# lazear/sage

Hardware: NVIDIA H100
Metric: spectra/sec (higher is better)
Workload: dtype f32

## Files before the change

sage_b200/csrc/device_common.cuh:

```cuda
#pragma once
#include <cuda_runtime.h>
#include <stdint.h>

namespace sb {

constexpr int K_MAX = 128;
constexpr uint32_t NARROW_CAP = 8192;
constexpr int PRELIM_THREADS = 256;
constexpr int SCORE_THREADS = 128;
#ifndef SAGE_B200_SCORE_MIN_CTAS
#define SAGE_B200_SCORE_MIN_CTAS 10
#endif
constexpr int SCORE_MIN_CTAS = SAGE_B200_SCORE_MIN_CTAS;
#ifndef SAGE_B200_SCORE_TILE
#define SAGE_B200_SCORE_TILE 1024
#endif
#ifndef SAGE_B200_SCORE_UNROLL
#define SAGE_B200_SCORE_UNROLL 1
#endif
#ifndef SAGE_B200_SCORE_MIN_CTAS_SPLIT
#define SAGE_B200_SCORE_MIN_CTAS_SPLIT 11
#endif
constexpr int SCORE_MIN_CTAS_SPLIT = SAGE_B200_SCORE_MIN_CTAS_SPLIT;
constexpr uint32_t SCORE_UNROLL = SAGE_B200_SCORE_UNROLL;
constexpr uint32_t SCORE_TILE = SAGE_B200_SCORE_TILE;
constexpr int MAX_KINDS = 6;
constexpr uint32_t WARPQ_CAP = 1024;
constexpr int WARPQ_WARPS = 2;
constexpr int WARPQ_MIN_CTAS = 24;
constexpr uint32_t PEP_LUT_CELLS = 65536;
constexpr uint32_t BUCKET_LUT_CELLS = 32768;

constexpr float PROTON = 1.0072764f;
constexpr float NEUTRON = 1.00335f;

struct Tol { int kind; float lo, hi; };

__device__ __forceinline__ int f32_key(float x) {
    int b = __float_as_int(x);
    return b ^ (int)(((unsigned)(b >> 31)) >> 1);
}

__device__ __forceinline__ float div_const_rn(float x, float c, float rc) {
    const float ax = fabsf(x);
    if (ax >= 1e-20f && ax <= 1e30f) {
        const float q0 = __fmul_rn(x, rc);
        return __fmaf_rn(__fmaf_rn(-q0, c, x), rc, q0);
    }
    return __fdiv_rn(x, c);
}

__device__ __forceinline__ void tol_bounds(const Tol& t, float c, float& lo, float& hi) {
    if (t.kind == 0) {
        lo = __fadd_rn(c, div_const_rn(__fmul_rn(c, t.lo), 1000000.0f, 1.0f / 1000000.0f));
        hi = __fadd_rn(c, div_const_rn(__fmul_rn(c, t.hi), 1000000.0f, 1.0f / 1000000.0f));
    } else if (t.kind == 1) {
        lo = __fadd_rn(c, div_const_rn(__fmul_rn(c, t.lo), 100.0f, 1.0f / 100.0f));
        hi = __fadd_rn(c, div_const_rn(__fmul_rn(c, t.hi), 100.0f, 1.0f / 100.0f));
    } else {
        lo = __fadd_rn(c, t.lo);
        hi = __fadd_rn(c, t.hi);
    }
// ... 65 lines not shown
    uint8_t mode;
};

struct QueryHits {
    uint32_t n;
    uint32_t default_run;
    uint32_t matched_peaks;
    uint32_t scored_candidates;
};

__device__ __forceinline__ uint32_t smem_u32(const void* p) { return (uint32_t)__cvta_generic_to_shared(p); }
__device__ __forceinline__ void mbar_init(uint64_t* bar, uint32_t count) {
    asm volatile("mbarrier.init.shared::cta.b64 [%0], %1;" ::"r"(smem_u32(bar)), "r"(count) : "memory");
    asm volatile("fence.mbarrier_init.release.cluster;" ::: "memory");
}
__device__ __forceinline__ void mbar_arrive_expect_tx(uint64_t* bar, uint32_t bytes) {
    asm volatile("mbarrier.arrive.expect_tx.shared::cta.b64 _, [%0], %1;" ::"r"(smem_u32(bar)), "r"(bytes) : "memory");
}
__device__ __forceinline__ void bulk_copy_g2s(void* dst_smem, const void* src_gmem, uint32_t bytes, uint64_t* bar) {
    asm volatile("cp.async.bulk.shared::cluster.global.mbarrier::complete_tx::bytes [%0], [%1], %2, [%3];" ::"r"(smem_u32(dst_smem)), "l"(src_gmem), "r"(bytes),
                 "r"(smem_u32(bar))
                 : "memory");
}
__device__ __forceinline__ void mbar_wait(uint64_t* bar, uint32_t parity) {
    uint32_t done = 0;
    while (!done) {
        asm volatile(
            "{\n\t.reg .pred p;\n\tmbarrier.try_wait.parity.shared::cta.b64 p, [%1], %2;\n\tselp.u32 %0, 1, 0, p;\n\t}"
            : "=r"(done)
            : "r"(smem_u32(bar)), "r"(parity)
            : "memory");
    }
}

struct ReplaySlot { unsigned long long off; uint32_t item, n_list, state , k; };

enum { C_TASKS = 0, C_PAGES, C_ENTRIES, C_MATCHED, C_CANDS, C_PEPFLOATS, C_PSMS, C_QUERIES, C_WIDE, C_MAXPOT, C_WORK, C_ERR, C_PEPQ, C_PEPFALLBACK, C_WSLOT, C_WOVERFLOW, C_FRAGS,
       C_NLIST , C_NCTA , C_NLIST_NEED ,
       C_HITS , C_COUNT };

struct DbView {
    const uint2* frag;
    const float* bucket_min;
    const float* pep_mono;
    const uint32_t* ion_off;
    const float* ions;
    const uint8_t* pep_len;
    const uint8_t* pep_flags;
    const uint8_t* pep_missed;
    uint32_t n_pep, n_bucket, bucket_size, n_kinds;
    uint32_t min_ion_index;
    uint32_t pep_centric_ok;
    uint32_t nterm_mask;
    const uint16_t* page_grid;
    uint32_t grid_shift, grid_n;
    const uint32_t* bucket_lut;
    float blut_base, blut_inv_w;
    const uint32_t* pep_lut;
    float plut_base, plut_inv_w;
    uint64_t n_frag;
    uint8_t kinds[MAX_KINDS];
};

struct WideIndexView {
    const uint2* frag;
    const uint64_t* blk_off;
// ... 54 lines not shown
```

sage_b200/csrc/kernels.cuh:

```cuda
#pragma once
#include <type_traits>

#include "device_common.cuh"
#include "glibc_log.cuh"

#ifndef SAGE_B200_RARE_NOINLINE
#define SAGE_B200_RARE_NOINLINE 0
#endif
#if SAGE_B200_RARE_NOINLINE
#define SB_RARE __noinline__
#else
#define SB_RARE __forceinline__
#endif

namespace sb {

__device__ __forceinline__ uint32_t pep_partition(const DbView& db, float x, bool le) {
    uint32_t lo = 0, hi = db.n_pep;
    if (db.pep_lut != nullptr) {
        const float t = (x - db.plut_base) * db.plut_inv_w;
        if (t == t) {
            const int c = (int)fminf(fmaxf(floorf(t), -2.0f), (float)PEP_LUT_CELLS + 2.0f);
            lo = __ldg(db.pep_lut + min(max(c - 1, 0), (int)PEP_LUT_CELLS));
            hi = __ldg(db.pep_lut + min(max(c + 2, 0), (int)PEP_LUT_CELLS));
// ... 229 lines not shown
}

__device__ __forceinline__ void index_probe(const DbView& db, const QueryDesc& q, float flo, float fhi, uint32_t* cnt32, uint32_t& matched, uint32_t& pages,
                                            uint32_t& entries) {
    uint32_t bl, br;
    bucket_range(db, flo, fhi, bl, br);
    for (uint32_t page = bl; page < br; page++) {
        const uint64_t pbase = (uint64_t)page * db.bucket_size;
        const uint64_t pend = min(pbase + db.bucket_size, db.n_frag);
        const uint2* slice = db.frag + pbase;
        const uint32_t pn = (uint32_t)(pend - pbase);
        const uint32_t pp = page_lower_bound_dir(db, page, slice, pn, q.pre_lo);
        const uint32_t il = pp == 0 ? 0 : pp - 1;
        uint32_t e = pp;
        for (; e < pn; e++) {
            const uint2 f = __ldg(&slice[e]);
            if (f.x > q.pre_hi) break;
            const float fmz = __uint_as_float(f.y);
            if (f.x >= q.eff_lo && f.x <= q.eff_hi && fmz >= flo && fmz <= fhi) {
                const uint32_t idx = f.x - q.pre_lo;
                atomicAdd(&cnt32[idx >> 1], 1u << ((idx & 1) * 16));
                matched++;
            }
        }
        pages++;
        entries += e - il;
    }
}

#ifndef SAGE_B200_WALK_SOLO
#define SAGE_B200_WALK_SOLO 8
#endif
constexpr uint32_t WALK_SOLO = SAGE_B200_WALK_SOLO;
__device__ __forceinline__ void block_probe_warp(const WideIndexView& nv, const QueryDesc& q, uint32_t b0, uint32_t b1, bool act, float flo, float fhi,
                                                 uint32_t* cnt32, uint32_t& matched) {
    const uint32_t lane = threadIdx.x & 31;
    const float tt = (flo - nv.base) * nv.inv_w;
    const int c = tt > 1.0f ? (int)fminf(tt, (float)(nv.cells - 1)) - 1 : 0;
    for (uint32_t blk = b0; blk <= b1; blk++) {
        const uint64_t base = __ldg(nv.blk_off + blk);
        const uint32_t cnt = (uint32_t)(__ldg(nv.blk_off + blk + 1) - base);
        const uint2* fr = nv.frag + base;
        uint32_t e = cnt;
        if (act) {
            e = __ldg(nv.lut + (size_t)blk * (nv.cells + 1) + c);
            for (uint32_t k = 0; k < WALK_SOLO && e < cnt; k++, e++) {
                const uint2 f = __ldg(fr + e);
                const float fmz = __uint_as_float(f.y);
                if (fmz > fhi) { e = cnt; break; }
                if (fmz >= flo && f.x >= q.eff_lo && f.x <= q.eff_hi) {
                    const uint32_t idx = f.x - q.pre_lo;
                    atomicAdd(&cnt32[idx >> 1], 1u << ((idx & 1) * 16));
                    matched++;
                }
            }
        }
        uint32_t pend = __ballot_sync(0xffffffffu, e < cnt);
        while (pend) {
            const int src = __ffs(pend) - 1;
            pend &= pend - 1;
            const uint32_t e0 = __shfl_sync(0xffffffffu, e, src);
            const float lo_s = __shfl_sync(0xffffffffu, flo, src), hi_s = __shfl_sync(0xffffffffu, fhi, src);
            for (uint32_t pos = e0; pos < cnt; pos += 32) {
                const uint32_t i = pos + lane;
                bool stop = i >= cnt;
                if (!stop) {
                    const uint2 f = __ldg(fr + i);
                    const float fmz = __uint_as_float(f.y);
                    stop = fmz > hi_s;
                    if (!stop && fmz >= lo_s && f.x >= q.eff_lo && f.x <= q.eff_hi) {
                        const uint32_t idx = f.x - q.pre_lo;
                        atomicAdd(&cnt32[idx >> 1], 1u << ((idx & 1) * 16));
                        matched++;
                    }
                }
                if (__any_sync(0xffffffffu, stop)) break;
            }
        }
    }
}

__device__ __forceinline__ void narrow_cta_query(const DbView& db, const ScorerView& sc, const BatchView& b, uint32_t pmax, uint64_t* nlist, uint32_t item,
                                                 float* bounds_smem, const WideIndexView& nv) {
    __shared__ uint32_t cnt32[NARROW_CAP / 2 + 1];
    __shared__ uint32_t s_warp[40];
    ReplaySlot* const nslots = b.nslots;
    const uint32_t s = item / sc.qmax;
    const QueryDesc q = b.queries[item];
    const uint32_t tid = threadIdx.x, lane = tid & 31, warp = tid >> 5, nwarps = PRELIM_THREADS / 32;
    const uint32_t p0 = b.peak_off[s], np = b.peak_off[s + 1] - p0;
    const uint32_t nwords = (q.potential + 1) >> 1;
    for (uint32_t i = tid; i < nwords; i += PRELIM_THREADS) cnt32[i] = 0;
    __shared__ unsigned long long s_loff;
    if (tid == 0 && q.potential > sc.kparam) s_loff = atomicAdd(b.counters + C_NLIST, (unsigned long long)q.potential);

    const uint32_t nfc = q.nfc;
    const uint32_t ntask = np * nfc;
    uint32_t my_matched = 0, my_pages = 0, my_entries = 0;
    __shared__ LutParams s_lp[8];
    bool pep_path = q.mode == 3 && np > 0 && np < 65536 && nfc <= 8;
    float* const bnd = bounds_smem;
    uint16_t* const luts = reinterpret_cast<uint16_t*>(bounds_smem + 2 * (size_t)nfc * pmax);
    if (pep_path) {
        for (uint32_t t = tid; t < ntask; t += PRELIM_THREADS) {
            const uint32_t c = t / np, p = t - c * np;
            const float mass = __fmul_rn(__ldg(b.masses + p0 + p), (float)(c + 1));
            float flo, fhi;
            tol_bounds(sc.fragment_tol, mass, flo, fhi);
            bnd[(2 * c) * pmax + p] = flo;
            bnd[(2 * c + 1) * pmax + p] = fhi;
        }
// ... 40 lines not shown
                            const float f = __ldg(src + j);
                            for (uint32_t c = 0; c < nfc; c++) {
                                const float* lo_c = bnd + (2 * c) * pmax;
                                const float* hi_c = lo_c + pmax;
                                const LutParams LP = s_lp[c];
                                uint32_t a = lut_start(LP, luts + (2 * c) * LUT_CELLS, f);
                                while (a < np && lo_c[a] <= f) a++;
                                uint32_t bb = lut_start(LP, luts + (2 * c + 1) * LUT_CELLS, f);
                                while (bb < a && hi_c[bb] < f) bb++;
                                c_here += a - min(bb, a);
                            }
                        }
                    }
                }
                for (int o = 16; o > 0; o >>= 1) c_here += __shfl_down_sync(0xffffffffu, c_here, o);
                if (lane == 0 && c_here) {
                    const uint32_t idx = pep - q.pre_lo;
                    atomicAdd(&cnt32[idx >> 1], (c_here & 0xFFFFu) << ((idx & 1) * 16));
                    my_matched += c_here;
                }
            }
        }
    } else if (nv.frag != nullptr) {
        const uint32_t blk0 = q.pre_lo / nv.block, blk1 = min(q.pre_hi, db.n_pep - 1) / nv.block;
        for (uint32_t t0 = warp * 32; t0 < ntask; t0 += PRELIM_THREADS) {
            const uint32_t t = t0 + lane;
            const bool act = t < ntask;
            float flo = 0.0f, fhi = 0.0f;
            if (act) {
                const uint32_t p = t / nfc, fc = t - p * nfc + 1;
                const float mass = __fmul_rn(__ldg(b.masses + p0 + p), (float)fc);
                tol_bounds(sc.fragment_tol, mass, flo, fhi);
            }
            block_probe_warp(nv, q, blk0, blk1, act, flo, fhi, cnt32, my_matched);
        }
    } else {
        for (uint32_t t = tid; t < ntask; t += PRELIM_THREADS) {
            const uint32_t p = t / nfc, fc = t - p * nfc + 1;
            const float mass = __fmul_rn(__ldg(b.masses + p0 + p), (float)fc);
            float flo, fhi;
            tol_bounds(sc.fragment_tol, mass, flo, fhi);
            index_probe(db, q, flo, fhi, cnt32, my_matched, my_pages, my_entries);
        }
    }
    __shared__ uint32_t s_red[3][PRELIM_THREADS / 32];
    {
        uint32_t a = my_matched, p = my_pages, en = my_entries;
        for (int o = 16; o > 0; o >>= 1) {
            a += __shfl_down_sync(0xffffffffu, a, o);
            p += __shfl_down_sync(0xffffffffu, p, o);
            en += __shfl_down_sync(0xffffffffu, en, o);
        }
        if (lane == 0) { s_red[0][warp] = a; s_red[1][warp] = p; s_red[2][warp] = en; }
    }
    __syncthreads();
    uint32_t matched_total = 0;
    for (uint32_t w = 0; w < nwarps; w++) matched_total += s_red[0][w];
    if (tid == 0) {
        uint32_t pages_total = 0, entries_total = 0;
        for (uint32_t w = 0; w < nwarps; w++) { pages_total += s_red[1][w]; entries_total += s_red[2][w]; }
        atomicAdd(b.counters + C_TASKS, (unsigned long long)ntask);
        if (pages_total) atomicAdd(b.counters + C_PAGES, (unsigned long long)pages_total);
        if (entries_total) atomicAdd(b.counters + C_ENTRIES, (unsigned long long)entries_total);
        atomicAdd(b.counters + C_MATCHED, (unsigned long long)matched_total);
    }
    QueryHits* h = b.hits + item;
    if (matched_total == 0) {
// ... 65 lines not shown
    const uint32_t total = (uint32_t)min(b.counters[C_NCTA], (unsigned long long)b.n * sc.qmax);
    for (uint32_t i = blockIdx.x; i < total; i += gridDim.x) {
        narrow_cta_query(db, sc, b, pmax, nlist, b.cta_items[i], bounds_smem, nv);
        __syncthreads();
    }
}

template <bool BLK>
__global__ void __launch_bounds__(WARPQ_WARPS * 32, WARPQ_MIN_CTAS) k_prelim_narrow_warp(DbView db, ScorerView sc, BatchView b, uint64_t* nlist, uint32_t s_lo,
                                                                                                uint32_t s_hi, WideIndexView nv) {
    __shared__ uint32_t cnt_all[WARPQ_WARPS][WARPQ_CAP / 2];
    if (b.counters[C_COUNT + blockIdx.y] == 0ull) return;
    const uint32_t lane = threadIdx.x & 31, warp = threadIdx.x >> 5;
    const uint32_t pos = blockIdx.x * WARPQ_WARPS + warp;
    if (pos >= b.n) return;
    const uint32_t s = b.order ? b.order[pos] : pos;
    if (s < s_lo || s >= s_hi) return;
    const uint32_t item = s * sc.qmax + blockIdx.y;
    const QueryDesc q = b.queries[item];
    if (q.mode != 4) return;
    uint32_t* const cnt32 = cnt_all[warp];
    const uint32_t n = q.potential, k = min(n, sc.kparam);
    for (uint32_t i = lane; i < (n + 1) >> 1; i += 32) cnt32[i] = 0;
    unsigned long long loff = 0;
    if (n > k) {
        if (lane == 0) loff = atomicAdd(b.counters + C_NLIST, (unsigned long long)n);
        loff = __shfl_sync(0xffffffffu, loff, 0);
    }
    __syncwarp();
    const uint32_t p0 = b.peak_off[s], np = b.peak_off[s + 1] - p0;
    const uint32_t nfc = q.nfc, ntask = np * nfc;
    uint32_t matched = 0, pages = 0, entries = 0;
    const uint32_t blk0 = BLK ? q.pre_lo / nv.block : 0u, blk1 = BLK ? min(q.pre_hi, db.n_pep - 1) / nv.block : 0u;
    for (uint32_t t0 = 0; t0 < ntask; t0 += 32) {
        const uint32_t t = t0 + lane;
        const bool act = t < ntask;
        float flo = 0.0f, fhi = 0.0f;
        if (act) {
            const uint32_t p = t / nfc, fc = t - p * nfc + 1;
            const float mass = __fmul_rn(__ldg(b.masses + p0 + p), (float)fc);
            tol_bounds(sc.fragment_tol, mass, flo, fhi);
        }
        if (BLK) block_probe_warp(nv, q, blk0, blk1, act, flo, fhi, cnt32, matched);
        else if (act) index_probe(db, q, flo, fhi, cnt32, matched, pages, entries);
    }
    for (int o = 16; o > 0; o >>= 1) {
        matched += __shfl_xor_sync(0xffffffffu, matched, o);
        pages += __shfl_xor_sync(0xffffffffu, pages, o);
        entries += __shfl_xor_sync(0xffffffffu, entries, o);
    }
    __syncwarp();
    if (lane == 0) {
        atomicAdd(b.counters + C_TASKS, (unsigned long long)ntask);
        if (pages) atomicAdd(b.counters + C_PAGES, (unsigned long long)pages);
        if (entries) atomicAdd(b.counters + C_ENTRIES, (unsigned long long)entries);
        if (matched) atomicAdd(b.counters + C_MATCHED, (unsigned long long)matched);
    }
    QueryHits* h = b.hits + item;
    ReplaySlot* slot = b.nslots + item;
    if (matched == 0 || (n > k && loff + n > b.nlist_cap)) {
        if (lane == 0) { h->n = 0; h->default_run = n; h->matched_peaks = 0; h->scored_candidates = 0; }
        return;
    }
    auto cnt = [&](uint32_t i) -> uint32_t { return (cnt32[i >> 1] >> ((i & 1) * 16)) & 0xFFFFu; };
    uint32_t nzc = 0;
    uint64_t* dst = n <= k ? b.hit_keys + (size_t)item * sc.kparam : nlist + loff;
    for (uint32_t i = lane; i < k; i += 32) {
        const uint32_t c = cnt(i);
        nzc += c != 0;
        dst[i] = c ? prescore_key(c, q.pre_lo + i, q.charge, q.iso) : PRESCORE_DEFAULT;
    }
    uint32_t wbase = k;
    for (uint32_t base = k; base < n; base += 32) {
        const uint32_t i = base + lane;
        const uint32_t c = i < n ? cnt(i) : 0;
        nzc += c != 0;
// ... 915 lines not shown
    float term[SCORE_TILE];
    float inten[SCORE_TILE];
    uint32_t mask[SCORE_TILE / 32];
    uint16_t hits[SCORE_TILE];
    uint16_t lut[SPEC_LUT_CELLS];
    uint32_t scan[SCORE_THREADS / 32];
    unsigned long long hit_base;
    uint32_t hit_room;
};

__device__ __forceinline__ uint32_t kind_index(uint32_t ki, uint32_t nions) {
    uint32_t kind = ki >= nions;
    uint32_t idx = ki - (kind ? nions : 0);
    while (idx >= nions) { idx -= nions; kind++; }
    return kind << 13 | idx;
}

__device__ __forceinline__ bool fast_task(float ion, uint32_t fc, float tlo, float thi, const SpecView& sp, const uint16_t* lut, const float* pm, float& mz,
                                          uint32_t& idx) {
    const float q3 = __fmul_rn(ion, 1.0f / 3.0f);
    const float third = __fmaf_rn(__fmaf_rn(-q3, 3.0f, ion), 1.0f / 3.0f, q3);
    mz = fc == 1 ? ion : (fc == 2 ? __fmul_rn(ion, 0.5f) : third);
    const float pl = __fmul_rn(mz, tlo), ph = __fmul_rn(mz, thi);
    const float ql = __fmul_rn(pl, 1.0f / 1000000.0f), qh = __fmul_rn(ph, 1.0f / 1000000.0f);
    const float lo = __fadd_rn(mz, __fmaf_rn(__fmaf_rn(-ql, 1000000.0f, pl), 1.0f / 1000000.0f, ql));
    const float hi = __fadd_rn(mz, __fmaf_rn(__fmaf_rn(-qh, 1000000.0f, ph), 1.0f / 1000000.0f, qh));
    const float tt = __fmul_rn(__fsub_rn(lo, sp.lp.base), sp.lp.inv_w);
    const int cc = tt > 1.0f ? (int)fminf(tt, (float)(SPEC_LUT_CELLS - 1)) - 1 : 0;
    idx = lut[cc];
    while (pm[idx] < lo) idx++;
    return pm[idx] <= hi;
}

template <bool FAST, bool SPLIT>
__device__ __forceinline__ void score_candidates_flat(const DbView& db, const ScorerView& sc, const uint64_t* cur, uint32_t ncand, const SpecView& sp,
                                                      ScoreTile& S, ScoreRec* recs, const SplitOut& so, uint32_t spec) {
    const uint32_t tid = threadIdx.x, lane = tid & 31, warp = tid >> 5, nwarps = SCORE_THREADS / 32;
    constexpr uint32_t tile = SCORE_TILE;
    uint64_t key = 0;
    uint32_t L = 0, nions = 0, nfc = 1, total = 0, ion_off = 0;
    if (tid < ncand) {
        key = cur[tid];
        const uint32_t pep = key_peptide(key);
        L = __ldg(db.pep_len + pep);
        nions = L - 1;
        nfc = max_fragment_charge(sc.max_fragment_charge_opt, key_charge(key)) - 1;
        total = nions * nfc * db.n_kinds;
        ion_off = __ldg(db.ion_off + pep);
    }
    uint32_t incl = total;
#pragma unroll
    for (int o = 1; o < 32; o <<= 1) {
        const uint32_t v = __shfl_up_sync(0xffffffffu, incl, o);
        if (lane >= (uint32_t)o) incl += v;
    }
    if (lane == 31) S.scan[warp] = incl;
    __syncthreads();
    uint32_t base = incl - total, T = 0;
#pragma unroll
    for (uint32_t w = 0; w < nwarps; w++) {
        const uint32_t x = S.scan[w];
        if (w < warp) base += x;
        T += x;
    }
    if (tid < ncand) { CandHdr h; h.ion_off = ion_off; h.base = base; h.next = base + total; h.nions = (uint16_t)nions; h.nfc = (uint8_t)nfc; h.pad = 0; S.hdr[tid] = h; }
    if (tid == 0) { CandHdr h; h.ion_off = 0; h.base = T; h.next = 0xFFFFFFFFu; h.nions = 0; h.nfc = 1; h.pad = 0; S.hdr[ncand] = h; }
    uint32_t hcnt = 0, hits_before = 0;
    if (SPLIT && tid == 0) {
        const unsigned long long hb = atomicAdd(so.counters + C_HITS, (unsigned long long)T);
        const bool room = hb + T <= so.hit_cap;
        S.hit_base = hb;
        S.hit_room = room ? 1u : 0u;
        so.meta[spec].hit_base = hb;
        if (!room) so.meta[spec].ncand = 0;
    }
    uint32_t mb = 0, my = 0;
    float sb = 0.f, sy = 0.f, ppm = 0.f;
    Run brun = {0, 0, 0, 0}, yrun = {0, 0, 0, 0};
    const float tlo = sc.fragment_tol.lo, thi = sc.fragment_tol.hi;
    const float* const pm = sp.masses;
    const float* const pi = sp.intens;
    auto generic_task = [&](const CandHdr& h, uint32_t f, uint32_t slot) -> bool {
        uint32_t ki, fc;
        switch (h.nfc) {
            case 1: ki = f; fc = 1; break;
            case 2: ki = f >> 1; fc = (f & 1) + 1; break;
            case 3: ki = f / 3; fc = f - ki * 3 + 1; break;
            default: ki = f / h.nfc; fc = f - ki * h.nfc + 1; break;
        }
        const float ion = __ldg(db.ions + h.ion_off + ki);
        const float mz = fc == 1 ? ion : (fc == 2 && fabsf(ion) >= 1e-30f) ? __fmul_rn(ion, 0.5f) : __fdiv_rn(ion, (float)fc);
        const int pk = sp.use_lut ? select_most_intense_peak_lut(pm, pi, sp.np, mz, sc.fragment_tol, sp.lp, S.lut)
                                  : select_most_intense_peak(pm, pi, sp.np, mz, sc.fragment_tol);
        if (pk < 0) return false;
        const float peak_mass = pm[pk], inten = pi[pk];
        S.term[slot] = __fdiv_rn(__fmul_rn(__fmul_rn(inten, fabsf(__fsub_rn(mz, peak_mass))), 2E6f), __fadd_rn(mz, peak_mass));
        S.inten[slot] = inten;
        return true;
    };
    for (uint32_t t0 = 0; t0 < T; t0 += tile) {
        const uint32_t tn = min(tile, T - t0);
        __syncthreads();
        PH(t0 == 0 ? 3 : 5);
        constexpr uint32_t STEP = 32 * SCORE_UNROLL;
        const uint32_t chunk = (((tn + nwarps - 1) / nwarps) + STEP - 1) & ~(STEP - 1);
        const uint32_t w_lo = min(tn, warp * chunk), w_hi = min(tn, w_lo + chunk);
        uint32_t c = 0, wcount = 0;
        CandHdr h = S.hdr[0];
        if (w_lo < w_hi) {
            const uint32_t t_first = t0 + min(w_lo + lane, w_hi - 1);
            uint32_t lo = 0, hi = ncand;
            while (hi - lo > 1) { const uint32_t mid = (lo + hi) >> 1; if (S.hdr[mid].base <= t_first) lo = mid; else hi = mid; }
            c = lo;
            h = S.hdr[c];
        }
        for (uint32_t s0 = w_lo; s0 < w_hi; s0 += STEP) {
            const uint32_t slotA = s0 + lane, slotB = slotA + 32;
            const bool inA = slotA < w_hi, inB = SCORE_UNROLL == 2 && slotB < w_hi;
            bool hitA = false, hitB = false, finalA = false, finalB = false;
            uint32_t fA = 0, fB = 0;
            CandHdr hA = h, hB = h;
            if (inA) {
                const uint32_t t = t0 + slotA;
                while (t >= h.next) { c++; h = S.hdr[c]; }
                hA = h; fA = t - h.base;
            }
            if (inB) {
                const uint32_t t = t0 + slotB;
                while (t >= h.next) { c++; h = S.hdr[c]; }
                hB = h; fB = t - h.base;
            }
            if (FAST) {
                const bool okA = inA && hA.nfc <= 3, okB = inB && hB.nfc <= 3;
                const uint32_t kiA = hA.nfc == 1 ? fA : (hA.nfc == 2 ? fA >> 1 : __umulhi(fA, 0xAAAAAAABu) >> 1);
                const uint32_t kiB = hB.nfc == 1 ? fB : (hB.nfc == 2 ? fB >> 1 : __umulhi(fB, 0xAAAAAAABu) >> 1);
                const float ionA = okA ? __ldg(db.ions + hA.ion_off + kiA) : 0.0f;
                const float ionB = okB ? __ldg(db.ions + hB.ion_off + kiB) : 0.0f;
                const bool fastA = okA && ionA >= 1.0f && ionA <= 1e20f, fastB = okB && ionB >= 1.0f && ionB <= 1e20f;
                float mzA = 0.f, mzB = 0.f;
                uint32_t idxA = 0, idxB = 0;
                if (fastA) hitA = fast_task(ionA, fA - kiA * hA.nfc + 1, tlo, thi, sp, S.lut, pm, mzA, idxA);
                if (fastB) hitB = fast_task(ionB, fB - kiB * hB.nfc + 1, tlo, thi, sp, S.lut, pm, mzB, idxB);
                if (hitA) { S.term[slotA] = mzA; S.inten[slotA] = __uint_as_float(idxA); }
                if (hitB) { S.term[slotB] = mzB; S.inten[slotB] = __uint_as_float(idxB); }
                if (inA && !fastA) hitA = finalA = generic_task(hA, fA, slotA);
                if (inB && !fastB) hitB = finalB = generic_task(hB, fB, slotB);
            } else {
                if (inA) hitA = generic_task(hA, fA, slotA);
                if (inB) hitB = generic_task(hB, fB, slotB);
            }
            const uint32_t ballA = __ballot_sync(0xffffffffu, hitA), ballB = __ballot_sync(0xffffffffu, hitB);
            if (lane == 0) { S.mask[s0 >> 5] = ballA; if (SCORE_UNROLL == 2) S.mask[(s0 >> 5) + 1] = ballB; }
            if (FAST) {
                const uint32_t lt = (1u << lane) - 1;
                if (hitA) S.hits[w_lo + wcount + __popc(ballA & lt)] = (uint16_t)(slotA | (finalA ? 0x8000u : 0u));
                wcount += __popc(ballA);
                if (SCORE_UNROLL == 2) {
                    if (hitB) S.hits[w_lo + wcount + __popc(ballB & lt)] = (uint16_t)(slotB | (finalB ? 0x8000u : 0u));
                    wcount += __popc(ballB);
                }
            }
        }
        if (FAST) {
            __syncwarp();
            for (uint32_t e = lane; e < wcount; e += 32) {
                const uint32_t ent = S.hits[w_lo + e];
                if (ent & 0x8000u) continue;
                const uint32_t slot = ent;
                const float mz = S.term[slot];
                uint32_t idx = __float_as_uint(S.inten[slot]);
                const float ph = __fmul_rn(mz, thi), qh = __fmul_rn(ph, 1.0f / 1000000.0f);
                const float hi = __fadd_rn(mz, __fmaf_rn(__fmaf_rn(-qh, 1000000.0f, ph), 1.0f / 1000000.0f, qh));
                int best = -1;
                float max_int = 0.0f;
                float m;
                do {
                    const float it = pi[idx];
                    if (it >= max_int) { max_int = it; best = (int)idx; }
                    m = pm[++idx];
                } while (m <= hi);
                if (best >= 0) {
                    const float peak_mass = pm[best];
                    S.term[slot] = __fdiv_rn(__fmul_rn(__fmul_rn(max_int, fabsf(__fsub_rn(mz, peak_mass))), 2E6f), __fadd_rn(mz, peak_mass));
                    S.inten[slot] = max_int;
                } else {
                    atomicAnd(&S.mask[slot >> 5], ~(1u << (slot & 31)));
                }
            }
        }
        __syncthreads();
        PH(4);
        if (SPLIT) {
            const uint32_t nwords = (tn + 31) >> 5;
// ... 58 lines not shown
                        switch (nfc) {
                            case 1: ki = f; break;
                            case 2: ki = f >> 1; break;
                            case 3: ki = f / 3; break;
                            default: ki = f / nfc; break;
                        }
                        uint32_t kind_i = ki >= nions;
                        uint32_t idx = ki - (kind_i ? nions : 0);
                        while (idx >= nions) { idx -= nions; kind_i++; }
                        const float it = S.inten[slot];
                        ppm = __fadd_rn(ppm, S.term[slot]);
                        if ((db.nterm_mask >> kind_i) & 1) { mb++; sb = __fadd_rn(sb, it); brun.matched(idx); }
                        else { my++; sy = __fadd_rn(sy, it); yrun.matched(idx); }
                    }
                }
            }
        }
    }
    if (SPLIT) {
        uint32_t inc2 = hcnt;
#pragma unroll
        for (int o = 1; o < 32; o <<= 1) {
            const uint32_t v = __shfl_up_sync(0xffffffffu, inc2, o);
            if (lane >= (uint32_t)o) inc2 += v;
        }
        __syncthreads();
        if (lane == 31) S.scan[warp] = inc2;
        __syncthreads();
        uint32_t h0 = inc2 - hcnt;
#pragma unroll
        for (uint32_t w = 0; w < nwarps; w++) if (w < warp) h0 += S.scan[w];
        if (tid < ncand) {
            CandOut co;
            co.key = key; co.h0 = h0; co.hcnt = hcnt; co.nions = (uint16_t)nions; co.nfc = (uint8_t)nfc; co.plen = (uint8_t)L; co.pad = 0;
            so.cand[(size_t)spec * sc.kparam + tid] = co;
        }
        return;
    }
    if (tid < ncand) {
        ScoreRec r;
        r.peptide = key_peptide(key); r.charge = key_charge(key); r.iso = key_iso(key);
        r.matched_b = mb & 0xFFFF; r.matched_y = my & 0xFFFF; r.summed_b = sb; r.summed_y = sy;
        r.longest_b = brun.longest; r.longest_y = yrun.longest;
        r.hyperscore = hyperscore_of(sc, r.matched_b, r.matched_y, sb, sy);
        r.ppm_difference = __fdiv_rn(ppm, __fadd_rn(sb, sy));
        r.valid = ((r.matched_b + r.matched_y) & 0xFFFF) >= sc.min_matched_peaks;
        r.plen = L;
        recs[tid] = r;
        S.hkey[tid] = r.valid ? r.hyperscore : -INFINITY;
    }
}

__device__ SB_RARE void annotate_candidate_warp(const DbView& db, const ScorerView& sc, uint32_t pep, uint32_t charge, const SpecView& sp,
                                                        FragmentOut* out, uint32_t cap_left) {
    const uint32_t lane = threadIdx.x & 31;
    const uint32_t L = __ldg(db.pep_len + pep);
    const uint32_t nions = L - 1;
    const uint32_t nfc = max_fragment_charge(sc.max_fragment_charge_opt, charge) - 1;
    const float* ions = db.ions + __ldg(db.ion_off + pep);
    const uint32_t total = nions * nfc * db.n_kinds;
    uint32_t written = 0;
    for (uint32_t base = 0; base < total; base += 32) {
        const uint32_t f = base + lane;
        int pk = -1;
        float mz = 0.f;
        uint32_t idx = 0, kind_i = 0, fc = 1;
        if (f < total) {
            const uint32_t ki = f / nfc;
            fc = f - ki * nfc + 1;
            idx = ki;
            while (idx >= nions) { idx -= nions; kind_i++; }
            mz = __fdiv_rn(__ldg(ions + ki), (float)fc);
            pk = sp.use_lut ? select_most_intense_peak_lut(sp.masses, sp.intens, sp.np, mz, sc.fragment_tol, sp.lp, sp.lut)
                            : select_most_intense_peak(sp.masses, sp.intens, sp.np, mz, sc.fragment_tol);
        }
        const uint32_t ball = __ballot_sync(0xffffffffu, pk >= 0);
        if (pk >= 0) {
            const uint32_t pos = written + __popc(ball & ((1u << lane) - 1));
            if (pos < cap_left) {
                const bool is_n = (db.nterm_mask >> kind_i) & 1;
// ... 15 lines not shown
    bool bad = np == 0 || np >= 65536;
    for (uint32_t i = threadIdx.x; i < np; i += blockDim.x) {
        const float m = masses[i];
        bad |= !(m > 0.0f) || (i > 0 && !(m >= masses[i - 1]));
    }
    if (__syncthreads_or(bad)) return false;
    lp = lut_params(masses[0], masses[np - 1], SPEC_LUT_CELLS);
    lut_build_walk(masses, np, lp, lut, threadIdx.x, blockDim.x, SPEC_LUT_CELLS);
    __syncthreads();
    return true;
}

template <bool SPLIT>
__global__ void __launch_bounds__(SCORE_THREADS, SPLIT ? SCORE_MIN_CTAS_SPLIT : SCORE_MIN_CTAS) k_score(DbView db, ScorerView sc, BatchView b, FeatureOut* features, uint32_t* counts, uint32_t pmax,
                                                         uint64_t* dbg_keys , uint32_t* dbg_meta, FragmentOut* frag_out ,
                                                         unsigned long long frag_cap, uint32_t quick_mode ,
                                                         uint8_t* keep , SplitOut so) {
    extern __shared__ __align__(16) unsigned char smem_raw[];
    float* masses_raw = reinterpret_cast<float*>(smem_raw);
    float* intens_raw = masses_raw + pmax + 4;
    uint64_t* cur = reinterpret_cast<uint64_t*>(intens_raw + pmax + 4);
    uint64_t* tot = cur + sc.lcap;
    ScoreRec* recs = reinterpret_cast<ScoreRec*>(tot + sc.lcap);
    uint32_t* order = reinterpret_cast<uint32_t*>(recs + sc.kparam);
    uint8_t* mark = reinterpret_cast<uint8_t*>(order + sc.kparam);
    __shared__ __align__(16) ScoreTile S;
    uint16_t* const lut = S.lut;
    __shared__ uint32_t s_ntot, s_ncand, s_np, s_nvalid;
    __shared__ unsigned long long s_matched_peaks, s_scored;
    __shared__ float s_tic;

    const uint32_t s = b.order ? b.order[blockIdx.x] : blockIdx.x, tid = threadIdx.x, lane = tid & 31, warp = tid >> 5, nwarps = SCORE_THREADS / 32;
    PH_START();
    const uint32_t p0 = b.peak_off[s];
    uint32_t np = b.peak_off[s + 1] - p0;
    __shared__ __align__(8) uint64_t s_bar;
    const uint32_t a0 = p0 & ~3u, head = p0 - a0;
    const uint32_t bytes = ((head + np) * 4 + 15) & ~15u;
    float* masses = masses_raw + head;
    float* intens = intens_raw + head;
    if (tid == 0) {
        mbar_init(&s_bar, 1);
        if (np) {
            mbar_arrive_expect_tx(&s_bar, 2 * bytes);
            bulk_copy_g2s(masses_raw, b.masses + a0, bytes, &s_bar);
            bulk_copy_g2s(intens_raw, b.intens + a0, bytes, &s_bar);
        }
    }

    const QueryDesc* qd = b.queries + (size_t)s * sc.qmax;
    const QueryHits* qh = b.hits + (size_t)s * sc.qmax;
    const uint64_t* qk = b.hit_keys + (size_t)s * sc.qmax * sc.kparam;
    const bool iso_fold = sc.min_iso != sc.max_iso;
    const bool single = !iso_fold && (sc.qmax == 1 || qd[1].mode == 0) && qd[0].mode != 0;
    if (single) {
        const QueryHits h = qh[0];
        const uint32_t n = h.n ? h.n : min(h.default_run, sc.kparam);
        for (uint32_t i = tid; i < n; i += SCORE_THREADS) tot[i] = h.n ? qk[i] : PRESCORE_DEFAULT;
        __syncthreads();
        if (warp == 0) {
            uint32_t w = 0;
            for (uint32_t base = 0; base < n; base += 32) {
                const uint32_t i = base + lane;
                const uint64_t k = i < n ? tot[i] : PRESCORE_DEFAULT;
                const bool keep = i < n && key_peptide(k) != 0xFFFFFFFFu;
                const uint32_t ball = __ballot_sync(0xffffffffu, keep);
                if (keep) cur[w + __popc(ball & ((1u << lane) - 1))] = k;
                w += __popc(ball);
            }
            if (lane == 0) { s_ntot = n; s_ncand = w; s_matched_peaks = h.matched_peaks; s_scored = h.scored_candidates; s_np = np; s_tic = b.tic[s]; }
        }
    } else if (tid == 0) {
        unsigned long long mp = 0, scd = 0;
        uint32_t ntot = 0;
        uint32_t nq = 0;
        while (nq < sc.qmax && qd[nq].mode != 0) nq++;
        const uint32_t nch = sc.n_iso ? nq / sc.n_iso : 0;
        for (uint32_t ci = 0; ci < nch; ci++) {
            uint32_t ncur = 0;
            for (uint32_t ii = 0; ii < sc.n_iso; ii++) {
                const uint32_t qi = ci * sc.n_iso + ii;
                mp += qh[qi].matched_peaks;
                scd += qh[qi].scored_candidates;
                ncur = append_hits(cur, ncur, sc.lcap, qh[qi], qk + (size_t)qi * sc.kparam, sc.kparam);
            }
            if (iso_fold) {
                const uint32_t k = min(ncur, sc.kparam);
                bounded_min_heapify_seq(cur, ncur, k);
                ncur = k;
            }
            for (uint32_t i = 0; i < ncur && ntot < sc.lcap; i++) tot[ntot++] = cur[i];
        }
        {
            const uint32_t k = min(ntot, sc.kparam);
            bounded_min_heapify_seq(tot, ntot, k);
            ntot = k;
        }
        s_ntot = ntot;
        s_matched_peaks = mp;
        s_scored = scd;
        uint32_t nc = 0;
        for (uint32_t i = 0; i < ntot; i++)
            if (key_peptide(tot[i]) != 0xFFFFFFFFu) cur[nc++] = tot[i];
        s_ncand = nc;
        s_np = np;
        s_tic = b.tic[s];
    }
    __syncthreads();
    PH(0);
    if (dbg_keys != nullptr) {
        for (uint32_t i = tid; i < s_ntot; i += SCORE_THREADS) dbg_keys[(size_t)s * sc.kparam + i] = tot[i];
        if (tid == 0) { dbg_meta[s * 4 + 0] = s_ntot; dbg_meta[s * 4 + 1] = (uint32_t)s_matched_peaks; dbg_meta[s * 4 + 2] = (uint32_t)s_scored; }
    }
    if (np) mbar_wait(&s_bar, 0);
    PH(1);
    if (tid == 0) masses[np] = INFINITY;
    const uint32_t ncand = s_ncand;
    if (SPLIT && tid == 0) {
        SpecMeta m;
        m.hit_base = 0; m.matched_peaks = s_matched_peaks; m.scored = s_scored; m.ncand = ncand; m.pad = 0;
        so.meta[s] = m;
    }
    const bool lists_fit = b.counters[C_NLIST_NEED] <= b.nlist_cap && b.counters[C_WIDE] <= (unsigned long long)b.wide_cap;
    if (quick_mode != 0 && !lists_fit) return;
    if (quick_mode == 1) {
        for (uint32_t i = tid; i < ncand; i += SCORE_THREADS) keep[key_peptide(cur[i])] = 1;
        return;
    }
    const float mzp = __fsub_rn(b.prec_mz[s], PROTON);
    const double lambda = (double)s_matched_peaks / (double)s_scored;
    const uint32_t rounds = sc.chimera ? sc.report_psms : 1;
    const uint32_t per_round = sc.chimera ? 1 : sc.report_psms;
    uint32_t nout = 0;
    SpecView sv;
    sv.masses = masses; sv.intens = intens; sv.lut = lut;
    for (uint32_t round = 0; round < rounds && ncand; round++) {
        np = s_np;
        sv.np = np;
        sv.use_lut = spectrum_lut_setup(masses, np, lut, sv.lp);
        PH(2);
        if (tid == 0) s_nvalid = 0;
        if (sv.use_lut && sc.score_fast && sc.fragment_tol.kind == 0 && fast_tol_ok(sc.fragment_tol.lo) && fast_tol_ok(sc.fragment_tol.hi))
            score_candidates_flat<true, SPLIT>(db, sc, cur, ncand, sv, S, recs, so, s);
        else
            score_candidates_flat<false, SPLIT>(db, sc, cur, ncand, sv, S, recs, so, s);
        if (SPLIT) return;
        __syncthreads();
        PH(5);
        if (quick_mode == 2) {
            if (tid < ncand && recs[tid].valid) {
                const uint32_t pme = recs[tid].peptide;
                uint32_t pos = 0;
                for (uint32_t j = 0; j < ncand; j++) {
                    if (!recs[j].valid) continue;
                    const uint32_t pj = recs[j].peptide;
                    pos += (pj > pme) || (pj == pme && j < tid);
                }
                if (pos < sc.report_psms) keep[pme] = 1;
            }
            return;
        }
        uint32_t my_floats = 0;
        if (tid < ncand) {
            my_floats = 2 * recs[tid].plen + 2;
            if (recs[tid].valid) {
                const double h = S.hkey[tid];
                uint32_t pos = 0;
                for (uint32_t j = 0; j < ncand; j++) {
                    const double hj = S.hkey[j];
                    pos += (hj > h) || (hj == h && j < tid);
                }
                order[pos] = tid;
                atomicAdd(&s_nvalid, 1u);
            }
        }
        if (tid < ((ncand + 31) & ~31u)) {
            for (int o = 16; o > 0; o >>= 1) my_floats += __shfl_down_sync(0xffffffffu, my_floats, o);
            if (lane == 0 && my_floats) atomicAdd(b.counters + C_PEPFLOATS, (unsigned long long)my_floats);
        }
// ... 602 lines not shown
```

Measured before the change: 23.17 million.

## Pair block probes, prefetch fragments and peak masses in warp-query kernel

Splits the per-block fragment walk into a helper and adds a paired variant that issues LUT and first-fragment loads for two index blocks before walking either, so their global-memory latencies overlap. The solo walk loop now prefetches the next fragment ahead of processing. The warp-query kernel also prefetches the next iteration's peak mass, and the default min-CTAs for warp-query launch bounds drops from 24 to 20, allowing more registers per thread. Together these trade extra registers and some code complexity for more memory-level parallelism.

```diff
diff --git a/sage_b200/csrc/device_common.cuh b/sage_b200/csrc/device_common.cuh
--- a/sage_b200/csrc/device_common.cuh
+++ b/sage_b200/csrc/device_common.cuh
@@ -27,7 +27,10 @@
 constexpr int MAX_KINDS = 6;
 constexpr uint32_t WARPQ_CAP = 1024;
 constexpr int WARPQ_WARPS = 2;
-constexpr int WARPQ_MIN_CTAS = 24;
+#ifndef SAGE_B200_WARPQ_MIN_CTAS
+#define SAGE_B200_WARPQ_MIN_CTAS 20
+#endif
+constexpr int WARPQ_MIN_CTAS = SAGE_B200_WARPQ_MIN_CTAS;
 constexpr uint32_t PEP_LUT_CELLS = 65536;
 constexpr uint32_t BUCKET_LUT_CELLS = 32768;
 
diff --git a/sage_b200/csrc/kernels.cuh b/sage_b200/csrc/kernels.cuh
--- a/sage_b200/csrc/kernels.cuh
+++ b/sage_b200/csrc/kernels.cuh
@@ -285,29 +285,20 @@
 #define SAGE_B200_WALK_SOLO 8
 #endif
 constexpr uint32_t WALK_SOLO = SAGE_B200_WALK_SOLO;
-__device__ __forceinline__ void block_probe_warp(const WideIndexView& nv, const QueryDesc& q, uint32_t b0, uint32_t b1, bool act, float flo, float fhi,
-                                                 uint32_t* cnt32, uint32_t& matched) {
+__device__ __forceinline__ void block_walk_warp(const uint2* fr, uint32_t cnt, uint32_t e, uint2 f, const QueryDesc& q, float flo, float fhi,
+                                                uint32_t* cnt32, uint32_t& matched) {
     const uint32_t lane = threadIdx.x & 31;
-    const float tt = (flo - nv.base) * nv.inv_w;
-    const int c = tt > 1.0f ? (int)fminf(tt, (float)(nv.cells - 1)) - 1 : 0;
-    for (uint32_t blk = b0; blk <= b1; blk++) {
-        const uint64_t base = __ldg(nv.blk_off + blk);
-        const uint32_t cnt = (uint32_t)(__ldg(nv.blk_off + blk + 1) - base);
-        const uint2* fr = nv.frag + base;
-        uint32_t e = cnt;
-        if (act) {
-            e = __ldg(nv.lut + (size_t)blk * (nv.cells + 1) + c);
-            for (uint32_t k = 0; k < WALK_SOLO && e < cnt; k++, e++) {
-                const uint2 f = __ldg(fr + e);
-                const float fmz = __uint_as_float(f.y);
-                if (fmz > fhi) { e = cnt; break; }
-                if (fmz >= flo && f.x >= q.eff_lo && f.x <= q.eff_hi) {
-                    const uint32_t idx = f.x - q.pre_lo;
-                    atomicAdd(&cnt32[idx >> 1], 1u << ((idx & 1) * 16));
-                    matched++;
-                }
-            }
-        }
+    for (uint32_t k = 0; k < WALK_SOLO && e < cnt; k++) {
+        const float fmz = __uint_as_float(f.y);
+        if (fmz > fhi) { e = cnt; break; }
+        if (fmz >= flo && f.x >= q.eff_lo && f.x <= q.eff_hi) {
+            const uint32_t idx = f.x - q.pre_lo;
+            atomicAdd(&cnt32[idx >> 1], 1u << ((idx & 1) * 16));
+            matched++;
+        }
+        if (++e < cnt && k + 1 < WALK_SOLO) f = __ldg(fr + e);
+    }
+    {
         uint32_t pend = __ballot_sync(0xffffffffu, e < cnt);
         while (pend) {
             const int src = __ffs(pend) - 1;
@@ -330,6 +321,29 @@
                 if (__any_sync(0xffffffffu, stop)) break;
             }
         }
+    }
+}
+template <bool PAIR>
+__device__ __forceinline__ void block_probe_warp(const WideIndexView& nv, const QueryDesc& q, uint32_t b0, uint32_t b1, bool act, float flo, float fhi,
+                                                 uint32_t* cnt32, uint32_t& matched) {
+    const float tt = (flo - nv.base) * nv.inv_w;
+    const int c = tt > 1.0f ? (int)fminf(tt, (float)(nv.cells - 1)) - 1 : 0;
+    for (uint32_t blk = b0; blk <= b1; blk += PAIR ? 2 : 1) {
+        const bool two = PAIR && blk < b1;
+        const uint64_t base0 = __ldg(nv.blk_off + blk), base1 = __ldg(nv.blk_off + blk + 1);
+        const uint64_t end1 = two ? __ldg(nv.blk_off + blk + 2) : base1;
+        const uint32_t cnt0 = (uint32_t)(base1 - base0), cnt1 = (uint32_t)(end1 - base1);
+        const uint2 *fr0 = nv.frag + base0, *fr1 = nv.frag + base1;
+        uint32_t e0 = cnt0, e1 = cnt1;
+        uint2 f0 = make_uint2(0u, 0u), f1 = make_uint2(0u, 0u);
+        if (act) {
+            e0 = __ldg(nv.lut + (size_t)blk * (nv.cells + 1) + c);
+            if (two) e1 = __ldg(nv.lut + (size_t)(blk + 1) * (nv.cells + 1) + c);
+            if (e0 < cnt0) f0 = __ldg(fr0 + e0);
+            if (e1 < cnt1) f1 = __ldg(fr1 + e1);
+        }
+        block_walk_warp(fr0, cnt0, e0, f0, q, flo, fhi, cnt32, matched);
+        if (two) block_walk_warp(fr1, cnt1, e1, f1, q, flo, fhi, cnt32, matched);
     }
 }
 
@@ -436,7 +450,7 @@
                 const float mass = __fmul_rn(__ldg(b.masses + p0 + p), (float)fc);
                 tol_bounds(sc.fragment_tol, mass, flo, fhi);
             }
-            block_probe_warp(nv, q, blk0, blk1, act, flo, fhi, cnt32, my_matched);
+            block_probe_warp<false>(nv, q, blk0, blk1, act, flo, fhi, cnt32, my_matched);
         }
     } else {
         for (uint32_t t = tid; t < ntask; t += PRELIM_THREADS) {
@@ -568,16 +582,19 @@
     const uint32_t nfc = q.nfc, ntask = np * nfc;
     uint32_t matched = 0, pages = 0, entries = 0;
     const uint32_t blk0 = BLK ? q.pre_lo / nv.block : 0u, blk1 = BLK ? min(q.pre_hi, db.n_pep - 1) / nv.block : 0u;
+    float peak_next = lane < ntask ? __ldg(b.masses + p0 + lane / nfc) : 0.0f;
     for (uint32_t t0 = 0; t0 < ntask; t0 += 32) {
         const uint32_t t = t0 + lane;
         const bool act = t < ntask;
+        const float peak = peak_next;
+        if (t + 32 < ntask) peak_next = __ldg(b.masses + p0 + (t + 32) / nfc);
         float flo = 0.0f, fhi = 0.0f;
         if (act) {
             const uint32_t p = t / nfc, fc = t - p * nfc + 1;
-            const float mass = __fmul_rn(__ldg(b.masses + p0 + p), (float)fc);
+            const float mass = __fmul_rn(peak, (float)fc);
             tol_bounds(sc.fragment_tol, mass, flo, fhi);
         }
-        if (BLK) block_probe_warp(nv, q, blk0, blk1, act, flo, fhi, cnt32, matched);
+        if (BLK) block_probe_warp<true>(nv, q, blk0, blk1, act, flo, fhi, cnt32, matched);
         else if (act) index_probe(db, q, flo, fhi, cnt32, matched, pages, entries);
     }
     for (int o = 16; o > 0; o >>= 1) {
```

New measurement: 23.49 million, median of 6. +1.4%, better.

## Prefetch ion masses via cp.async and hoist query/candidate loads earlier

Applied to the files above, without the earlier changes.

Splits the per-tile scoring loop into two phases. First each lane issues cp.async 4-byte copies of the needed ion masses into shared memory along with a packed candidate/fragment index, then a second pass computes matches from shared memory. The query hit keys, the tic value and the per-candidate peptide length and ion offset are now loaded before the peak bulk-copy wait, so their latency overlaps it. The SCORE_UNROLL knob is removed. The cost is an extra shared-memory pass and a 24-bit packing of the fragment index, which assumes fewer than 256 candidates and 2^24 fragments per tile.

```diff
diff --git a/sage_b200/csrc/device_common.cuh b/sage_b200/csrc/device_common.cuh
--- a/sage_b200/csrc/device_common.cuh
+++ b/sage_b200/csrc/device_common.cuh
@@ -15,14 +15,10 @@
 #ifndef SAGE_B200_SCORE_TILE
 #define SAGE_B200_SCORE_TILE 1024
 #endif
-#ifndef SAGE_B200_SCORE_UNROLL
-#define SAGE_B200_SCORE_UNROLL 1
-#endif
 #ifndef SAGE_B200_SCORE_MIN_CTAS_SPLIT
 #define SAGE_B200_SCORE_MIN_CTAS_SPLIT 11
 #endif
 constexpr int SCORE_MIN_CTAS_SPLIT = SAGE_B200_SCORE_MIN_CTAS_SPLIT;
-constexpr uint32_t SCORE_UNROLL = SAGE_B200_SCORE_UNROLL;
 constexpr uint32_t SCORE_TILE = SAGE_B200_SCORE_TILE;
 constexpr int MAX_KINDS = 6;
 constexpr uint32_t WARPQ_CAP = 1024;
@@ -159,6 +155,11 @@
             : "memory");
     }
 }
+
+__device__ __forceinline__ void cp_async_4(void* dst_smem, const void* src_gmem) {
+    asm volatile("cp.async.ca.shared.global [%0], [%1], 4;" ::"r"(smem_u32(dst_smem)), "l"(src_gmem) : "memory");
+}
+__device__ __forceinline__ void cp_async_wait_all() { asm volatile("cp.async.wait_all;" ::: "memory"); }
 
 struct ReplaySlot { unsigned long long off; uint32_t item, n_list, state , k; };
 
diff --git a/sage_b200/csrc/kernels.cuh b/sage_b200/csrc/kernels.cuh
--- a/sage_b200/csrc/kernels.cuh
+++ b/sage_b200/csrc/kernels.cuh
@@ -1559,22 +1559,30 @@
     return pm[idx] <= hi;
 }
 
+struct CandLoad { uint32_t nions, ion_off, nfc; };
+__device__ __forceinline__ CandLoad load_candidate(const DbView& db, const ScorerView& sc, const uint64_t* cur, uint32_t ncand) {
+    CandLoad cl = {0, 0, 1};
+    if (threadIdx.x < ncand) {
+        const uint64_t key = cur[threadIdx.x];
+        const uint32_t pep = key_peptide(key);
+        cl.nions = __ldg(db.pep_len + pep) - 1u;
+        cl.ion_off = __ldg(db.ion_off + pep);
+        cl.nfc = max_fragment_charge(sc.max_fragment_charge_opt, key_charge(key)) - 1;
+    }
+    return cl;
+}
+
+__device__ __forceinline__ uint32_t task_ion(uint32_t f, uint32_t nfc) {
+    if (nfc > 3) return f / nfc;
+    return nfc == 1 ? f : (nfc == 2 ? f >> 1 : __umulhi(f, 0xAAAAAAABu) >> 1);
+}
+
 template <bool FAST, bool SPLIT>
-__device__ __forceinline__ void score_candidates_flat(const DbView& db, const ScorerView& sc, const uint64_t* cur, uint32_t ncand, const SpecView& sp,
-                                                      ScoreTile& S, ScoreRec* recs, const SplitOut& so, uint32_t spec) {
+__device__ __forceinline__ void score_candidates_flat(const DbView& db, const ScorerView& sc, const uint64_t* cur, const CandLoad& cl, uint32_t ncand,
+                                                      const SpecView& sp, ScoreTile& S, ScoreRec* recs, const SplitOut& so, uint32_t spec) {
     const uint32_t tid = threadIdx.x, lane = tid & 31, warp = tid >> 5, nwarps = SCORE_THREADS / 32;
     constexpr uint32_t tile = SCORE_TILE;
-    uint64_t key = 0;
-    uint32_t L = 0, nions = 0, nfc = 1, total = 0, ion_off = 0;
-    if (tid < ncand) {
-        key = cur[tid];
-        const uint32_t pep = key_peptide(key);
-        L = __ldg(db.pep_len + pep);
-        nions = L - 1;
-        nfc = max_fragment_charge(sc.max_fragment_charge_opt, key_charge(key)) - 1;
-        total = nions * nfc * db.n_kinds;
-        ion_off = __ldg(db.ion_off + pep);
-    }
+    const uint32_t nions = cl.nions, nfc = cl.nfc, ion_off = cl.ion_off, total = nions * nfc * db.n_kinds;
     uint32_t incl = total;
 #pragma unroll
     for (int o = 1; o < 32; o <<= 1) {
@@ -1607,15 +1615,14 @@
     const float tlo = sc.fragment_tol.lo, thi = sc.fragment_tol.hi;
     const float* const pm = sp.masses;
     const float* const pi = sp.intens;
-    auto generic_task = [&](const CandHdr& h, uint32_t f, uint32_t slot) -> bool {
-        uint32_t ki, fc;
-        switch (h.nfc) {
-            case 1: ki = f; fc = 1; break;
-            case 2: ki = f >> 1; fc = (f & 1) + 1; break;
-            case 3: ki = f / 3; fc = f - ki * 3 + 1; break;
-            default: ki = f / h.nfc; fc = f - ki * h.nfc + 1; break;
-        }
-        const float ion = __ldg(db.ions + h.ion_off + ki);
+    auto generic_task = [&](uint32_t nfc_, uint32_t f, float ion, uint32_t slot) -> bool {
+        uint32_t fc;
+        switch (nfc_) {
+            case 1: fc = 1; break;
+            case 2: fc = (f & 1) + 1; break;
+            case 3: fc = f - (f / 3) * 3 + 1; break;
+            default: fc = f - (f / nfc_) * nfc_ + 1; break;
+        }
         const float mz = fc == 1 ? ion : (fc == 2 && fabsf(ion) >= 1e-30f) ? __fmul_rn(ion, 0.5f) : __fdiv_rn(ion, (float)fc);
         const int pk = sp.use_lut ? select_most_intense_peak_lut(pm, pi, sp.np, mz, sc.fragment_tol, sp.lp, S.lut)
                                   : select_most_intense_peak(pm, pi, sp.np, mz, sc.fragment_tol);
@@ -1629,63 +1636,49 @@
         const uint32_t tn = min(tile, T - t0);
         __syncthreads();
         PH(t0 == 0 ? 3 : 5);
-        constexpr uint32_t STEP = 32 * SCORE_UNROLL;
-        const uint32_t chunk = (((tn + nwarps - 1) / nwarps) + STEP - 1) & ~(STEP - 1);
+        const uint32_t chunk = (((tn + nwarps - 1) / nwarps) + 31) & ~31u;
         const uint32_t w_lo = min(tn, warp * chunk), w_hi = min(tn, w_lo + chunk);
-        uint32_t c = 0, wcount = 0;
-        CandHdr h = S.hdr[0];
-        if (w_lo < w_hi) {
-            const uint32_t t_first = t0 + min(w_lo + lane, w_hi - 1);
+        if (w_lo + lane < w_hi) {
+            const uint32_t t_first = t0 + w_lo + lane;
             uint32_t lo = 0, hi = ncand;
             while (hi - lo > 1) { const uint32_t mid = (lo + hi) >> 1; if (S.hdr[mid].base <= t_first) lo = mid; else hi = mid; }
-            c = lo;
-            h = S.hdr[c];
-        }
-        for (uint32_t s0 = w_lo; s0 < w_hi; s0 += STEP) {
-            const uint32_t slotA = s0 + lane, slotB = slotA + 32;
-            const bool inA = slotA < w_hi, inB = SCORE_UNROLL == 2 && slotB < w_hi;
-            bool hitA = false, hitB = false, finalA = false, finalB = false;
-            uint32_t fA = 0, fB = 0;
-            CandHdr hA = h, hB = h;
-            if (inA) {
-                const uint32_t t = t0 + slotA;
+            uint32_t c = lo;
+            CandHdr h = S.hdr[c];
+            for (uint32_t slot = w_lo + lane; slot < w_hi; slot += 32) {
+                const uint32_t t = t0 + slot;
                 while (t >= h.next) { c++; h = S.hdr[c]; }
-                hA = h; fA = t - h.base;
-            }
-            if (inB) {
-                const uint32_t t = t0 + slotB;
-                while (t >= h.next) { c++; h = S.hdr[c]; }
-                hB = h; fB = t - h.base;
-            }
+                const uint32_t f = t - h.base;
+                cp_async_4(&S.term[slot], db.ions + h.ion_off + task_ion(f, h.nfc));
+                S.inten[slot] = __uint_as_float(c << 24 | f);
+            }
+            cp_async_wait_all();
+        }
+        uint32_t wcount = 0;
+        for (uint32_t s0 = w_lo; s0 < w_hi; s0 += 32) {
+            const uint32_t slot = s0 + lane;
+            bool hit = false, fin = false;
+            if (slot < w_hi) {
+                const uint32_t cf = __float_as_uint(S.inten[slot]), f = cf & 0xFFFFFFu;
+                const uint32_t hnfc = S.hdr[cf >> 24].nfc;
+                const float ion = S.term[slot];
+                if (FAST) {
+                    if (hnfc <= 3 && ion >= 1.0f && ion <= 1e20f) {
+                        float mz;
+                        uint32_t idx;
+                        hit = fast_task(ion, f - task_ion(f, hnfc) * hnfc + 1, tlo, thi, sp, S.lut, pm, mz, idx);
+                        if (hit) { S.term[slot] = mz; S.inten[slot] = __uint_as_float(idx); }
+                    } else {
+                        hit = fin = generic_task(hnfc, f, ion, slot);
+                    }
+                } else {
+                    hit = generic_task(hnfc, f, ion, slot);
+                }
+            }
+            const uint32_t ball = __ballot_sync(0xffffffffu, hit);
+            if (lane == 0) S.mask[s0 >> 5] = ball;
             if (FAST) {
-                const bool okA = inA && hA.nfc <= 3, okB = inB && hB.nfc <= 3;
-                const uint32_t kiA = hA.nfc == 1 ? fA : (hA.nfc == 2 ? fA >> 1 : __umulhi(fA, 0xAAAAAAABu) >> 1);
-                const uint32_t kiB = hB.nfc == 1 ? fB : (hB.nfc == 2 ? fB >> 1 : __umulhi(fB, 0xAAAAAAABu) >> 1);
-                const float ionA = okA ? __ldg(db.ions + hA.ion_off + kiA) : 0.0f;
-                const float ionB = okB ? __ldg(db.ions + hB.ion_off + kiB) : 0.0f;
-                const bool fastA = okA && ionA >= 1.0f && ionA <= 1e20f, fastB = okB && ionB >= 1.0f && ionB <= 1e20f;
-                float mzA = 0.f, mzB = 0.f;
-                uint32_t idxA = 0, idxB = 0;
-                if (fastA) hitA = fast_task(ionA, fA - kiA * hA.nfc + 1, tlo, thi, sp, S.lut, pm, mzA, idxA);
-                if (fastB) hitB = fast_task(ionB, fB - kiB * hB.nfc + 1, tlo, thi, sp, S.lut, pm, mzB, idxB);
-                if (hitA) { S.term[slotA] = mzA; S.inten[slotA] = __uint_as_float(idxA); }
-                if (hitB) { S.term[slotB] = mzB; S.inten[slotB] = __uint_as_float(idxB); }
-                if (inA && !fastA) hitA = finalA = generic_task(hA, fA, slotA);
-                if (inB && !fastB) hitB = finalB = generic_task(hB, fB, slotB);
-            } else {
-                if (inA) hitA = generic_task(hA, fA, slotA);
-                if (inB) hitB = generic_task(hB, fB, slotB);
-            }
-            const uint32_t ballA = __ballot_sync(0xffffffffu, hitA), ballB = __ballot_sync(0xffffffffu, hitB);
-            if (lane == 0) { S.mask[s0 >> 5] = ballA; if (SCORE_UNROLL == 2) S.mask[(s0 >> 5) + 1] = ballB; }
-            if (FAST) {
-                const uint32_t lt = (1u << lane) - 1;
-                if (hitA) S.hits[w_lo + wcount + __popc(ballA & lt)] = (uint16_t)(slotA | (finalA ? 0x8000u : 0u));
-                wcount += __popc(ballA);
-                if (SCORE_UNROLL == 2) {
-                    if (hitB) S.hits[w_lo + wcount + __popc(ballB & lt)] = (uint16_t)(slotB | (finalB ? 0x8000u : 0u));
-                    wcount += __popc(ballB);
-                }
+                if (hit) S.hits[w_lo + wcount + __popc(ball & ((1u << lane) - 1))] = (uint16_t)(slot | (fin ? 0x8000u : 0u));
+                wcount += __popc(ball);
             }
         }
         if (FAST) {
@@ -1810,20 +1803,21 @@
         for (uint32_t w = 0; w < nwarps; w++) if (w < warp) h0 += S.scan[w];
         if (tid < ncand) {
             CandOut co;
-            co.key = key; co.h0 = h0; co.hcnt = hcnt; co.nions = (uint16_t)nions; co.nfc = (uint8_t)nfc; co.plen = (uint8_t)L; co.pad = 0;
+            co.key = cur[tid]; co.h0 = h0; co.hcnt = hcnt; co.nions = (uint16_t)nions; co.nfc = (uint8_t)nfc; co.plen = (uint8_t)(nions + 1); co.pad = 0;
             so.cand[(size_t)spec * sc.kparam + tid] = co;
         }
         return;
     }
     if (tid < ncand) {
         ScoreRec r;
+        const uint64_t key = cur[tid];
         r.peptide = key_peptide(key); r.charge = key_charge(key); r.iso = key_iso(key);
         r.matched_b = mb & 0xFFFF; r.matched_y = my & 0xFFFF; r.summed_b = sb; r.summed_y = sy;
         r.longest_b = brun.longest; r.longest_y = yrun.longest;
         r.hyperscore = hyperscore_of(sc, r.matched_b, r.matched_y, sb, sy);
         r.ppm_difference = __fdiv_rn(ppm, __fadd_rn(sb, sy));
         r.valid = ((r.matched_b + r.matched_y) & 0xFFFF) >= sc.min_matched_peaks;
-        r.plen = L;
+        r.plen = nions + 1;
         recs[tid] = r;
         S.hkey[tid] = r.valid ? r.hyperscore : -INFINITY;
     }
@@ -1905,6 +1899,23 @@
 
     const uint32_t s = b.order ? b.order[blockIdx.x] : blockIdx.x, tid = threadIdx.x, lane = tid & 31, warp = tid >> 5, nwarps = SCORE_THREADS / 32;
     PH_START();
+    const QueryDesc* qd = b.queries + (size_t)s * sc.qmax;
+    const QueryHits* qh = b.hits + (size_t)s * sc.qmax;
+    const uint64_t* qk = b.hit_keys + (size_t)s * sc.qmax * sc.kparam;
+    const bool iso_fold = sc.min_iso != sc.max_iso;
+    const uint32_t mode0 = qd[0].mode, mode1 = (!iso_fold && sc.qmax > 1) ? qd[1].mode : 0;
+    QueryHits h0 = {0, 0, 0, 0};
+    uint64_t keys0[K_MAX / 32];
+    float tic = 0.0f;
+    if (warp == 0) {
+        h0 = qh[0];
+        tic = b.tic[s];
+#pragma unroll
+        for (uint32_t j = 0; j < K_MAX / 32; j++) {
+            const uint32_t i = j * 32 + lane;
+            keys0[j] = i < sc.kparam ? qk[i] : PRESCORE_DEFAULT;
+        }
+    }
     const uint32_t p0 = b.peak_off[s];
     uint32_t np = b.peak_off[s + 1] - p0;
     __shared__ __align__(8) uint64_t s_bar;
@@ -1921,27 +1932,22 @@
         }
     }
 
-    const QueryDesc* qd = b.queries + (size_t)s * sc.qmax;
-    const QueryHits* qh = b.hits + (size_t)s * sc.qmax;
-    const uint64_t* qk = b.hit_keys + (size_t)s * sc.qmax * sc.kparam;
-    const bool iso_fold = sc.min_iso != sc.max_iso;
-    const bool single = !iso_fold && (sc.qmax == 1 || qd[1].mode == 0) && qd[0].mode != 0;
+    const bool single = !iso_fold && mode1 == 0 && mode0 != 0;
     if (single) {
-        const QueryHits h = qh[0];
-        const uint32_t n = h.n ? h.n : min(h.default_run, sc.kparam);
-        for (uint32_t i = tid; i < n; i += SCORE_THREADS) tot[i] = h.n ? qk[i] : PRESCORE_DEFAULT;
-        __syncthreads();
         if (warp == 0) {
+            const uint32_t n = h0.n ? h0.n : min(h0.default_run, sc.kparam);
             uint32_t w = 0;
-            for (uint32_t base = 0; base < n; base += 32) {
-                const uint32_t i = base + lane;
-                const uint64_t k = i < n ? tot[i] : PRESCORE_DEFAULT;
+#pragma unroll
+            for (uint32_t j = 0; j < K_MAX / 32; j++) {
+                const uint32_t i = j * 32 + lane;
+                const uint64_t k = h0.n ? keys0[j] : PRESCORE_DEFAULT;
                 const bool keep = i < n && key_peptide(k) != 0xFFFFFFFFu;
                 const uint32_t ball = __ballot_sync(0xffffffffu, keep);
                 if (keep) cur[w + __popc(ball & ((1u << lane) - 1))] = k;
                 w += __popc(ball);
-            }
-            if (lane == 0) { s_ntot = n; s_ncand = w; s_matched_peaks = h.matched_peaks; s_scored = h.scored_candidates; s_np = np; s_tic = b.tic[s]; }
+                if (dbg_keys != nullptr && i < n) tot[i] = k;
+            }
+            if (lane == 0) { s_ntot = n; s_ncand = w; s_matched_peaks = h0.matched_peaks; s_scored = h0.scored_candidates; s_np = np; s_tic = tic; }
         }
     } else if (tid == 0) {
         unsigned long long mp = 0, scd = 0;
@@ -1977,10 +1983,12 @@
             if (key_peptide(tot[i]) != 0xFFFFFFFFu) cur[nc++] = tot[i];
         s_ncand = nc;
         s_np = np;
-        s_tic = b.tic[s];
+        s_tic = tic;
     }
     __syncthreads();
     PH(0);
+    const uint32_t ncand = s_ncand;
+    const CandLoad cl = load_candidate(db, sc, cur, ncand);
     if (dbg_keys != nullptr) {
         for (uint32_t i = tid; i < s_ntot; i += SCORE_THREADS) dbg_keys[(size_t)s * sc.kparam + i] = tot[i];
         if (tid == 0) { dbg_meta[s * 4 + 0] = s_ntot; dbg_meta[s * 4 + 1] = (uint32_t)s_matched_peaks; dbg_meta[s * 4 + 2] = (uint32_t)s_scored; }
@@ -1988,7 +1996,6 @@
     if (np) mbar_wait(&s_bar, 0);
     PH(1);
     if (tid == 0) masses[np] = INFINITY;
-    const uint32_t ncand = s_ncand;
     if (SPLIT && tid == 0) {
         SpecMeta m;
         m.hit_base = 0; m.matched_peaks = s_matched_peaks; m.scored = s_scored; m.ncand = ncand; m.pad = 0;
@@ -2014,10 +2021,10 @@
         PH(2);
         if (tid == 0) s_nvalid = 0;
         if (sv.use_lut && sc.score_fast && sc.fragment_tol.kind == 0 && fast_tol_ok(sc.fragment_tol.lo) && fast_tol_ok(sc.fragment_tol.hi))
-            score_candidates_flat<true, SPLIT>(db, sc, cur, ncand, sv, S, recs, so, s);
+            score_candidates_flat<true, SPLIT>(db, sc, cur, cl, ncand, sv, S, recs, so, s);
         else
-            score_candidates_flat<false, SPLIT>(db, sc, cur, ncand, sv, S, recs, so, s);
-        if (SPLIT) return;
+            score_candidates_flat<false, SPLIT>(db, sc, cur, cl, ncand, sv, S, recs, so, s);
+        if (SPLIT) { PH(5); return; }
         __syncthreads();
         PH(5);
         if (quick_mode == 2) {
```

New measurement: 23.06 million before, 23.97 million after, median of 6. +4.0%, better.
